# PlantandFoodResearch/MCHap

Measured on AMD Instinct MI355X. Metric: loci/sec (whole node) for 1000-step MCMC, tetraploid 8-SNV loci, 1/2/4/8 GPUs, higher is better.
Workload: dtype f64; 1 GPU; 10000 synthetic tetraploid loci per GPU, 8 SNVs, 200 reads, 1000 MCMC steps x 2 chains, burn 500, posterior summary (BASELINE.json configs[1]); 4 passes in flight on separate HIP streams, each with its own device buffers; loci_per_gpu=10000, ploidy=4, snvs=8, reads=200, mcmc_steps=1000, chains=2, burn=500, llk_cache=True, passes_in_flight=4, hw_queues=4, world_size=1, devices=1

## Files before the change

include/mchap_hip.h:

```cpp
#ifndef MCHAP_HIP_H
#define MCHAP_HIP_H

#include <stdint.h>
#include <stddef.h>

#ifdef __cplusplus
extern "C" {
#endif

#define MCHAP_MAX_TEMPS 16
#define MCHAP_MAX_PLOIDY 8
#define MCHAP_MAX_PLOIDY_DENOVO 15
#define MCHAP_MAX_POS 126
#define MCHAP_MAX_ALLELE 8
#define MCHAP_MAX_READS 4096

enum {
  MCHAP_OK = 0,
  MCHAP_ERR_NAN_LLK = -1,
  MCHAP_ERR_BAD_ARG = -2,
  MCHAP_ERR_BREAKS = -3,
  MCHAP_ERR_LIMIT = -4,
  MCHAP_ERR_HIP = -5,
  MCHAP_ERR_NO_DEVICE = -6
// ... 57 lines not shown
  uint64_t stream_id;
  int32_t initial_n_het;
  int32_t reserved;
} mchap_unit;

int mchap_denovo_fit_batch_device(const mchap_denovo_cfg *cfg, int n_units, const mchap_unit *units_dev,
                                  const mchap_unit *units_host, const double *reads, const int64_t *read_counts,
                                  const int8_t *n_alleles, const int8_t *initial, uint64_t *trace_words,
                                  double *llks, int8_t *fixed_alleles, int32_t *status, void *workspace,
                                  int64_t workspace_bytes, void *stream);

int mchap_denovo_fit_batch_calls_device(const mchap_denovo_cfg *cfg, int n_units, const mchap_unit *units_dev,
                                        const mchap_unit *units_host, const int8_t *calls, const int16_t *quals,
                                        const double *qual_prob, int qual_prob_len, const int64_t *read_counts,
                                        const int8_t *n_alleles, const int8_t *initial, uint64_t *trace_words,
                                        double *llks, int8_t *fixed_alleles, int32_t *status, void *workspace,
                                        int64_t workspace_bytes, void *stream);

int64_t mchap_denovo_workspace_bytes(const mchap_denovo_cfg *cfg, int n_units, const mchap_unit *units_host);

int mchap_denovo_fit_batch(const mchap_denovo_cfg *cfg, int n_units, const mchap_unit *units,
                           const double *reads, int64_t reads_len, const int64_t *read_counts, int64_t counts_len,
                           const int8_t *n_alleles, int64_t nalleles_len, const int8_t *initial, int64_t initial_len,
                           uint64_t *trace_words, int64_t trace_len, double *llks, int64_t llks_len,
                           int8_t *fixed_alleles, int64_t fixed_len, int32_t *status);

int mchap_log_likelihood_batch(const double *reads, int n_reads, int n_pos, int max_allele,
                               const int64_t *read_counts, const int8_t *genotypes, int n_genotypes, int ploidy,
                               double *llks_out);

int mchap_read_log_batch(const double *x, int64_t n, double *out);
int mchap_read_log_product_batch(const double *x, int64_t n, int group, double *out);
int mchap_wave_sum_batch(const double *x, int64_t n_waves, double *out);

int mchap_trace_posterior_batch_device(int n_units, const mchap_unit *units_dev, int steps, int chains, int burn,
                                       const uint64_t *trace_words, int max_states, int ploidy_max,
                                       uint64_t *post_words, int32_t *post_counts, int32_t *post_n,
                                       double *mode_stats, int32_t *mode_index, uint64_t *mode_words,
                                       int32_t *mode_count, void *stream);

int mchap_trace_posterior_max_states(int ploidy_max);
int mchap_trace_posterior_listed_device(int n_list, const int32_t *unit_list_dev, const mchap_unit *units_dev, int steps, int chains,
                                        int burn, const uint64_t *trace_words, int cap, int ploidy_max, uint64_t *post_words,
                                        int32_t *post_counts, int32_t *post_n, double *mode_stats, int32_t *mode_index,
                                        uint64_t *mode_words, int32_t *mode_count, void *stream);

int mchap_call_incongruence_batch_device(int n_units, const mchap_unit *units_dev, int steps, int chains, int burn,
                                         const int64_t *genotypes, int ploidy_max, double threshold, int32_t *mci, void *stream);
int mchap_call_incongruence_listed_device(int n_list, const int32_t *unit_list_dev, const mchap_unit *units_dev, int steps, int chains,
                                          int burn, const int64_t *genotypes, int cap, int ploidy_max, double threshold, int32_t *mci,
                                          void *stream);

int mchap_exact_genotype_likelihoods(const double *reads, int n_reads, int n_pos, int max_allele,
                                     const int64_t *read_counts, const int8_t *haplotypes, int n_haps, int ploidy,
                                     float *llks_out, double *llks64_out);

int mchap_exact_genotype_posteriors(const void *llks, int is_f32, int64_t n_genotypes, int ploidy, int n_alleles,
                                    int has_prior, double inbreeding, const double *frequencies, double *post_out);

int mchap_trace_incongruence_batch_device(int n_units, const mchap_unit *units_dev, int steps, int chains, int burn,
                                          const uint64_t *trace_words, int ploidy_max, double threshold, int32_t *mci,
                                          void *stream);

int mchap_trace_incongruence_listed_device(int n_list, const int32_t *unit_list_dev, const mchap_unit *units_dev, int steps, int chains,
                                           int burn, const uint64_t *trace_words, int cap, int ploidy_max, double threshold, int32_t *mci,
                                           void *stream);
// ... 97 lines not shown
```

mchap_amd/_lib.py:

```python
import ctypes as C
import os
import threading
import subprocess

import numpy as np

HERE = os.path.dirname(os.path.abspath(__file__))
CSRC = os.path.join(HERE, "csrc")
SO = os.environ.get("MCHAP_HIP_LIB") or os.path.join(CSRC, "libmchap_hip.so")
TEST_SO = os.path.join(CSRC, "libmchap_hip_test.so")

MAX_TEMPS = 16
MAX_PLOIDY = 8
MAX_PLOIDY_GENERAL = 15
MAX_ALLELE = 8
MAX_READS = 4096

OK = 0
ERR_NAN_LLK = -1
ERR_BAD_ARG = -2
ERR_BREAKS = -3
ERR_LIMIT = -4
ERR_HIP = -5
ERR_NO_DEVICE = -6
# ... 213 lines not shown
    "mchap_trace_posterior_batch_wph_device",
    "mchap_trace_posterior_max_states_wph",
    "mchap_trace_posterior_listed_wph_device",
    "mchap_trace_incongruence_batch_wph_device",
    "mchap_trace_incongruence_listed_wph_device",
    "mchap_call_incongruence_batch_device",
    "mchap_call_incongruence_listed_device",
    "mchap_exact_genotype_likelihoods",
    "mchap_exact_genotype_posteriors",
    "mchap_exact_posterior_mode_batch",
    "mchap_exact_workspace_bytes",
    "mchap_exact_workspace_bytes_cached",
    "mchap_exact_call_batch_device",
    "mchap_exact_posterior_summaries_batch_device",
    "mchap_exact_posterior_summaries",
    "mchap_call_mcmc_workspace_bytes",
    "mchap_call_mcmc_workspace_bytes_for",
    "mchap_call_mcmc_max_haps",
    "mchap_call_mcmc_batch_device",
    "mchap_call_mcmc_batch",
    "mchap_call_reads_from_calls_device",
    "mchap_version",
    "mchap_last_error",
    "mchap_device_count",
    "mchap_denovo_lds_bytes",
    "mchap_denovo_workspace_bytes",
    "mchap_timer_create",
    "mchap_timer_ms",
    "mchap_timer_destroy",
    "mchap_denovo_sampler_name",
    "mchap_read_log_batch",
    "mchap_read_log_product_batch",
    "mchap_wave_sum_batch",
    "mchap_denovo_trace_words_per_haplotype",
]


def last_error():
    return lib().mchap_last_error().decode()


def check(rc):
    if rc == OK:
        return
    msg = last_error()
    if rc == ERR_NAN_LLK:
        raise ValueError("Encountered log likelihood of nan")
    if rc == ERR_BREAKS:
        raise ValueError("breaks must be smaller then n")
    if rc == ERR_BAD_ARG:
        raise AssertionError(msg)
    if rc == ERR_LIMIT:
        raise NotImplementedError("mchap_hip: " + msg)
    raise MchapLibraryError("mchap_hip error %d: %s" % (rc, msg))


def ptr(a):
    return None if a is None else C.c_void_p(a.ctypes.data)
```

mchap_amd/csrc/denovo_coast_kernel.hpp:

```cpp
#pragma once
#include "denovo_spec_kernel.hpp"

namespace mchap {

template <int NW>
__device__ __forceinline__ void coast_chain(const SimtParams &P, unsigned char *smem, int slot) {
  const DenovoParams &D = P.d;
  const int tid = threadIdx.x;
  const int lane = tid & (WAVE - 1), wv = tid / WAVE;
  constexpr int NT = NW * WAVE;
  auto block_sync = [] {
    if constexpr (NW == 1) lds_sync();
    else __syncthreads();
  };
  const int Cn = D.chains, Sn = D.steps, mmax = P.max_pos;
  const int E = spec_memo_entries(mmax);
  const long long q = P.pipe_list ? (long long)P.pipe_list[slot] : (long long)slot;
  PipeState *st = reinterpret_cast<PipeState *>(P.pipe_state) + q;
  const int base = st->step;
  if (base >= Sn) return;
  const int u = (int)(q / Cn), chain = (int)(q % Cn);
  const mchap_unit U = D.units[u];
  const int32_t *mi = P.meta_i + (size_t)u * meta_i_stride(P.max_pos);
  const int K = U.ploidy;
  const int Mh = mi[META_I_MH];
  const int n = K * Mh;
  if (st->mvalid == 0 || n > spec_draws(K, mmax)) {
    if (tid == 0) P.pipe_out[atomicAdd(P.pipe_out_count, 1)] = (int32_t)q;
    return;
  }
  LDSP(double) mt = lds_cast<double>(smem);
  LDSP(double) bc = mt + 2 * E;
  LDSP(uint64_t) tw = lds_cast<uint64_t>(smem + (size_t)8 * (2 * E + mmax));
  LDSP(int) wfail = lds_cast<int>(smem + (size_t)8 * (2 * E + mmax + 8));
  const double mlo = st->mlo, mhi = st->mhi;
  {
    const double *pm = P.pipe_memo + (size_t)q * 2 * E;
    for (int i = tid; i < 2 * E; i += NT) mt[i] = pm[i];
  }
  if (tid == 0) {
    if (D.n_intervals == 0) {
      double cacc = 0.0;
      for (int j = 0; j < Mh; j++) {
        cacc += D.break_table[(size_t)Mh * D.max_pos + j];
        bc[j] = cacc;
      }
    }
    uint64_t w[8];
#pragma unroll
    for (int h = 0; h < 8; h++) w[h] = h < K ? st->g[h] : ~0ull;
#pragma unroll
    for (int pass = 0; pass < 8; pass++) {
#pragma unroll
      for (int i = pass & 1; i + 1 < 8; i += 2) {
        const uint64_t a = w[i], b = w[i + 1];
        w[i] = a < b ? a : b;
        w[i + 1] = a < b ? b : a;
      }
    }
#pragma unroll
    for (int h = 0; h < 8; h++) tw[h] = w[h];
  }
  block_sync();
  Stream s;
  s.k0 = (uint32_t)D.seed;
  s.k1 = (uint32_t)(D.seed >> 32) ^ (uint32_t)(U.stream_id >> 32);
  s.c2 = ((uint32_t)chain << 16) | 0u;
  s.c3 = (uint32_t)U.stream_id;
  int stop = Sn;
  int sweep = 0;
  for (int s0 = base; s0 < Sn; s0 += NT, sweep++) {
    const int step = s0 + tid;
    bool fail = false;
    if (step < Sn) {
      const uint64_t ctr0 = (uint64_t)step * STEP_DRAWS;
      const uint64_t ub = ctr0 + (uint64_t)(n - 1), ue = ub + (uint64_t)n;
      uint64_t dblk = ~0ull, dw0 = 0, dw1 = 0;
      auto words_at = [&](uint64_t d) -> uint64_t {
        const uint64_t b = d >> 1;
        if (b != dblk) {
          uint32_t o[4];
          philox4x32_10((uint32_t)b, (uint32_t)(b >> 32), s.c2, s.c3, s.k0, s.k1, o);
          dw0 = (uint64_t)o[0] | ((uint64_t)o[1] << 32);
          dw1 = (uint64_t)o[2] | ((uint64_t)o[3] << 32);
          dblk = b;
        }
        return (d & 1) ? dw1 : dw0;
      };
      bool ok = true;
      for (uint64_t b = ub >> 1; 2 * b < ue; b++) {
        uint32_t o[4];
        philox4x32_10((uint32_t)b, (uint32_t)(b >> 32), s.c2, s.c3, s.k0, s.k1, o);
        const uint64_t d0 = 2 * b;
        const uint64_t w0 = (uint64_t)o[0] | ((uint64_t)o[1] << 32), w1 = (uint64_t)o[2] | ((uint64_t)o[3] << 32);
        if (d0 >= ub && d0 < ue) {
          const double x = draw_double(w0);
          ok = ok && (mlo <= x) && (x < mhi);
        }
        if (d0 + 1 >= ub && d0 + 1 < ue) {
          const double x = draw_double(w1);
          ok = ok && (mlo <= x) && (x < mhi);
        }
        dblk = b;
        dw0 = w0;
        dw1 = w1;
      }
      fail = !ok;
      uint64_t ctr = ue;
      for (int kind = 0; kind < 3 && !fail; kind++) {
        const double pstep = kind == 0 ? D.p_recomb : (kind == 1 ? D.p_partial : D.p_dosage);
        const bool doit = draw_double(words_at(ctr)) <= pstep;
        ctr++;
        if (!doit) continue;
        uint64_t zeros;
        int n_int;
        if (kind < 2) {
          int nb;
          if (D.n_intervals > 0) {
            ctr++;
            nb = D.n_intervals - 1;
          } else {
            const double x = draw_double(words_at(ctr));
            ctr++;
            nb = Mh;
            for (int j = Mh - 1; j >= 0; j--)
              if (bc[j] > x) nb = j;
          }
          if (nb >= Mh) {
            fail = true;
            break;
          }
          uint64_t ind = ((1ull << Mh) - 1ull) & ~1ull;
          for (int b = 0; b < nb; b++) {
            const int no = __popcll(ind);
            if (no == 0) break;
            int k = 0;
            if (no > 1) {
              k = (int)draw_interval(words_at(ctr), (uint32_t)(no - 1));
              ctr++;
            }
            uint64_t t = ind;
            while (k-- > 0) t &= t - 1;
            ind &= ~(t & (~t + 1));
          }
          zeros = ~ind & ((1ull << (Mh + 1)) - 1ull);
          n_int = nb + 1;
        } else {
          zeros = 1ull | (1ull << Mh);
          n_int = 1;
        }
        LDSP(double) mtot = mt + (kind == 0 ? 0 : E);
        if (n_int == 1) {
          const double tot = mtot[spec_memo_index(0, Mh)];
          if (tot < 0.0) continue;
          if (!(draw_double(words_at(ctr)) >= tot)) {
            fail = true;
            break;
          }
          ctr++;
        } else {
          double mx = -1.0;
          int n_cons = 0;
          bool unknown = false;
          uint64_t z = zeros;
          int start = __ffsll((long long)z) - 1;
          z &= z - 1;
          for (int i = 0; i < n_int; i++) {
            const int stop_ = __ffsll((long long)z) - 1;
            z &= z - 1;
            const double tot = mtot[spec_memo_index(start, stop_)];
            if (isnan(tot)) unknown = true;
            else if (tot >= 0.0) {
              n_cons++;
              mx = fmax(mx, tot);
            }
            start = stop_;
          }
          bool low = unknown;
          for (int k = 0; k < n_cons && !low; k++)
            low = !(draw_double(words_at(ctr + (uint64_t)(n_int - 1 + k))) >= mx);
          if (low) {
            fail = true;
            break;
          }
          ctr += (uint64_t)(n_int - 1 + n_cons);
        }
      }
    }
    const unsigned long long fb = __ballot(fail);
    if constexpr (NW == 1) {
      if (fb) {
        stop = s0 + __ffsll((long long)fb) - 1;
        break;
      }
    } else {
      LDSP(int) wf = wfail + (sweep & 1) * NW;
      if (lane == 0) wf[wv] = fb ? s0 + wv * WAVE + __ffsll((long long)fb) - 1 : Sn;
      __syncthreads();
      int first = Sn;
#pragma unroll
      for (int w = 0; w < NW; w++) first = min(first, wf[w]);
      if (first < Sn) {
        stop = first;
        break;
      }
    }
  }
  if (tid == 0) {
    st->step = stop;
    if (stop < Sn) P.pipe_out[atomicAdd(P.pipe_out_count, 1)] = (int32_t)q;
  }
  const int rows = stop - base;
  uint64_t *tp = D.trace + U.trace_off + (size_t)chain * D.steps * K + (size_t)base * K;
  uint64_t *lp = reinterpret_cast<uint64_t *>(D.llks + U.llk_off + (size_t)chain * D.steps) + base;
  const int nw = rows * K;
  int h = tid % K;
  const int hs = NT % K;
  for (int i = tid; i < nw; i += NT) {
    tp[i] = tw[h];
// ... 23 lines not shown
```

mchap_amd/csrc/denovo_spec_kernel.hpp:

```cpp
#pragma once
#include <type_traits>

#include "denovo_simt_kernel.hpp"

#ifdef MCHAP_MASK_PADDING
#define MCHAP_PAD_LANE(x) (x)
#else
#define MCHAP_PAD_LANE(x) true
#endif
#ifndef MCHAP_COOP_UNR
#define MCHAP_COOP_UNR 2
#endif
#ifndef MCHAP_SPEC_TB
#define MCHAP_SPEC_TB 4
#endif
#ifndef MCHAP_SPEC_LOW
#define MCHAP_SPEC_LOW 8
#endif
#ifndef MCHAP_SPEC_CG
#define MCHAP_SPEC_CG 4
#endif
#ifndef MCHAP_SPEC_VAR
#define MCHAP_SPEC_VAR 0
#endif
#define MCHAP_SPEC_SBS (MCHAP_SPEC_VAR == 1)
#define MCHAP_SPEC_DEEP (MCHAP_SPEC_VAR == 2)
#ifndef MCHAP_SPEC_WIN0
#define MCHAP_SPEC_WIN0 4
#endif
#ifndef MCHAP_SPEC_WIN_MIN
#define MCHAP_SPEC_WIN_MIN 2
#endif
#ifndef MCHAP_REUSE_MAXK
#define MCHAP_REUSE_MAXK 8
#endif
#ifndef MCHAP_CODED_UNR
#define MCHAP_CODED_UNR 16
#endif

namespace mchap {

constexpr int SPEC_MAX_IV = 64;
constexpr int SPEC_TB = MCHAP_SPEC_TB;
constexpr int SPEC_LN = 72;
constexpr int SPEC_DRAWS_MAX = 384;
__host__ __device__ inline int spec_draws(int K, int Mmax) {
  int d = 2 * K * Mmax - 1;
  if (d < 3 * Mmax + 2) d = 3 * Mmax + 2;
  d = (d + 1) & ~1;
  return d < SPEC_DRAWS_MAX ? d : SPEC_DRAWS_MAX;
}

#define LDSP(T) __attribute__((address_space(3))) T *
#define GLBP(T) __attribute__((address_space(1))) T *
template <class T>
__device__ __forceinline__ LDSP(T) lds_cast(void *p) {
  return (LDSP(T))p;
}

template <bool LT>
struct TabPtr;
template <>
struct TabPtr<false> {
  typedef GLBP(const uint8_t) u8;
  typedef GLBP(const double) f64;
  template <class CT>
  static __device__ __forceinline__ CT ld(u8 p) { return *reinterpret_cast<GLBP(const CT)>(p); }
};
template <>
struct TabPtr<true> {
  typedef LDSP(const uint8_t) u8;
  typedef LDSP(const double) f64;
  template <class CT>
  static __device__ __forceinline__ CT ld(u8 p) { return *reinterpret_cast<LDSP(const CT)>(p); }
};

enum { GP_RT = 0, GP_CW, GP_CT, GP_CACHE, GP_CKEYS, GP_TRACE, GP_LLK, GP_GBP, GP_N };
// ... 59 lines not shown
  const size_t per_group = (size_t)2 * spec_memo_entries(Mmax) * 8;
  if (T != 1 || per_group > 16 * 1024) return 0;
  return per_group * (64 / G);
}

constexpr int SPEC_LC_ENTRIES = 256;
#ifndef MCHAP_LC_GEN
#define MCHAP_LC_GEN 48
#endif
constexpr uint32_t SPEC_LC_SECOND_LEVEL_GEN = MCHAP_LC_GEN;
__host__ __device__ inline size_t spec_lc_bytes(int entries = SPEC_LC_ENTRIES) { return (size_t)16 * entries + 16; }
__host__ __device__ inline bool spec_ctx_in_bpc(int K, int Mmax, int Amax, int max_reads) {
  return K >= 3 && max_reads <= 64 && Mmax * Amax <= 24 * (K - 2) && 16 * K * Mmax <= 3 * 64 * 8 && 12 * 64 + 4 * 8 <= 3 * 64 * 8;
}
__host__ __device__ inline int spec_lc_entries(int bp_cache) { return (bp_cache & 2) ? ((bp_cache & 4) ? SPEC_LC_ENTRIES / 2 : SPEC_LC_ENTRIES) : 0; }
__device__ __forceinline__ uint32_t sct_off(uint32_t row) { return (row / 24u) * (uint32_t)(4 * WAVE * 8) + (row % 24u) * (uint32_t)WAVE; }
__host__ __device__ inline size_t spec_bp_cache_bytes(int K) { return (size_t)8 * K * 4 * 64 + (size_t)8 * (K + 1); }

constexpr int COAST_NW_LIST = 4;
__host__ __device__ inline size_t coast_lds_bytes(int Mmax) {
  return (size_t)8 * (2 * spec_memo_entries(Mmax) + Mmax) + (size_t)8 * 12;
}

__host__ __device__ inline size_t spec_lds_bytes(int K, int Mmax, int Amax, int T, int G) {
  const int NG = 64 / G;
  const int nmax = K * Mmax;
  const int nopt = Amax > 1 ? Amax - 1 : 1;
  const int niv = Mmax + 1;
  size_t b = 0;
  b += (size_t)8 * K * 64;
  b += (size_t)8 * NG * T * K;
  b += (size_t)8 * NG * T * 2;
  b += (size_t)8 * NG * (2 * K + 5);
  b += (size_t)8 * 64;
  b += (size_t)8 * nopt * 64 * 2;
  b += (size_t)8 * SPEC_LN * 2;
  b += (size_t)8 * NG * Mmax;
  b += (size_t)4 * NG * niv * 4;
  b += (size_t)2 * NG * Mmax;
  b += (size_t)2 * NG * nmax;
  b += (size_t)NG * Mmax * 2;
  b += (size_t)NG * nmax;
  b += (size_t)NG * niv;
  b = (b + 1) & ~(size_t)1;
  b += (size_t)2 * NG * 2;
  b = (b + 15) & ~(size_t)15;
  b += (size_t)8 * NG * DICT_MAX;
  b += (size_t)8 * NG * GP_N;
  b += (size_t)8 * NG * GV_N;
  b = (b + 15) & ~(size_t)15;
  b += (size_t)16 * NG;
  b += (size_t)8 * NG * K;
  b += (size_t)8 * NG * (K + 1);
  b += (size_t)8 * NG * SPEC_TB * (K + 1);
  b = (b + 15) & ~(size_t)15;
  b += (size_t)8 * NG * spec_draws(K, Mmax);
  b += spec_memo_bytes(Mmax, T, G);
  return (b + 63) & ~(size_t)63;
}

struct Stream {
  uint32_t k0, k1, c2, c3;
};
__device__ __forceinline__ void stream_words(const Stream &s, uint64_t n, uint32_t &a, uint32_t &b) {
  uint32_t o[4];
  const uint64_t blk = n >> 1;
  philox4x32_10((uint32_t)blk, (uint32_t)(blk >> 32), s.c2, s.c3, s.k0, s.k1, o);
  a = (n & 1) ? o[2] : o[0];
  b = (n & 1) ? o[3] : o[1];
}
__device__ __forceinline__ double stream_double(const Stream &s, uint64_t n) {
  uint32_t a, b;
  stream_words(s, n, a, b);
  return ((double)(a >> 5) * 67108864.0 + (double)(b >> 6)) * (1.0 / 9007199254740992.0);
}
__device__ __forceinline__ uint32_t stream_interval(const Stream &s, uint64_t n, uint32_t max) {
  uint32_t a, b;
  stream_words(s, n, a, b);
  return __umulhi(a, max + 1u);
}

template <int G>
__device__ __forceinline__ void stage_draws(const Stream &s, uint64_t base, int count, LDSP(uint64_t) tab, int gl, bool active) {
  if (active) {
    const uint64_t b0 = base >> 1;
    const int nblk = (int)(((base + (uint64_t)count + 1) >> 1) - b0);
    for (int b = gl; b < nblk; b += G) {
      uint32_t o[4];
      const uint64_t blk = b0 + (uint64_t)b;
      philox4x32_10((uint32_t)blk, (uint32_t)(blk >> 32), s.c2, s.c3, s.k0, s.k1, o);
      const long long i0 = (long long)(blk << 1) - (long long)base;
      if (i0 >= 0 && i0 < count) tab[i0] = (uint64_t)o[0] | ((uint64_t)o[1] << 32);
      if (i0 + 1 >= 0 && i0 + 1 < count) tab[i0 + 1] = (uint64_t)o[2] | ((uint64_t)o[3] << 32);
    }
  }
}
__device__ __forceinline__ double draw_double(uint64_t w) {
  return ((double)((uint32_t)w >> 5) * 67108864.0 + (double)((uint32_t)(w >> 32) >> 6)) * (1.0 / 9007199254740992.0);
}
__device__ __forceinline__ uint32_t draw_interval(uint64_t w, uint32_t max) { return __umulhi((uint32_t)w, max + 1u); }

template <int G>
__device__ __forceinline__ uint64_t grp_ballot(bool p, int gi) {
  const unsigned long long m = __ballot(p);
  if (G == 64) return m;
  return (m >> (gi * G)) & ((1ull << G) - 1ull);
}
__device__ __forceinline__ bool wave_any(bool p) { return __ballot(p) != 0ull; }

template <int CTRL>
__device__ __forceinline__ double dpp_f64(double v) {
  const long long b = __double_as_longlong(v);
  const int lo = __builtin_amdgcn_update_dpp(0, (int)(unsigned)b, CTRL, 0xf, 0xf, false);
  const int hi = __builtin_amdgcn_update_dpp(0, (int)(unsigned)((unsigned long long)b >> 32), CTRL, 0xf, 0xf, false);
  return __longlong_as_double((long long)(((unsigned long long)(unsigned)hi << 32) | (unsigned)lo));
}
template <int G>
__device__ __forceinline__ double grp_max_f64(double v) {
#pragma unroll
  for (int o = G / 2; o >= 16; o >>= 1) v = fmax(v, __shfl_xor(v, o, G));
  v = fmax(v, dpp_f64<0x128>(v));
  v = fmax(v, dpp_f64<0x124>(v));
  v = fmax(v, dpp_f64<0x122>(v));
  v = fmax(v, dpp_f64<0x121>(v));
  return v;
}
__device__ __forceinline__ void lds_sync() {
#ifdef MCHAP_SYNC_BARRIER
  __syncthreads();
#else
  __builtin_amdgcn_fence(__ATOMIC_ACQ_REL, "workgroup");
  __builtin_amdgcn_wave_barrier();
#endif
// ... 1889 lines not shown
          const int idx = spec_memo_index((int)(se & 255u), (int)(se >> 8));
          mtot[idx] = no > 0 ? cacc : -1.0;
          ctx_tot(idx, no > 0 ? cacc : -1.0);
        }
        off += no;
      }
      ii0 = ii;
    }
    {
      const int src = acc_gl >= 0 ? acc_gl : 0;
      GWords<KT> nw;
#pragma unroll
      for (int h = 0; h < KT; h++) nw.w[h] = __shfl(pw.w[h], src, G);
      const double nl = __shfl(llk_i, src, G);
      if (acc_gl >= 0) {
        c.g = nw;
        c.llk = nl;
        genotype_changed<KT>(c);
      }
    }
    if (!done && ii0 >= n_int) done = true;
    lds_sync();
  }
  } while (fill && wave_any(filling && n_int > 0));
  GPHASE(c, 7);
  return ok;
}



constexpr int SPEC_TW_MAX = 8;
__host__ __device__ inline size_t spec_tw_exchange_bytes(int K, int T) { return (((size_t)8 * T * (K + 1) + 16) + 63) & ~(size_t)63; }

template <int KT, int G, bool PIPE = false, int VAR = MCHAP_SPEC_VAR, bool TW = false, bool CTX = false>
__global__ __launch_bounds__(TW ? 64 * SPEC_TW_MAX : 64, TW ? 2 : MCHAP_SPEC_WPE) void denovo_spec_kernel(const SimtParams P) {
  extern __shared__ __align__(16) unsigned char smem_all[];
  constexpr int NG = 64 / G;
  const DenovoParams &D = P.d;
  const int lane = threadIdx.x & (WAVE - 1);
  const int tw = TW ? (int)(threadIdx.x / WAVE) : 0;
  unsigned char *smem = smem_all + (TW ? spec_tw_exchange_bytes(KT, D.n_temps) + (size_t)tw * (size_t)P.tw_lds : 0);
  LDSP(uint64_t) xw = lds_cast<uint64_t>(smem_all);
  LDSP(double) xllk = lds_cast<double>(smem_all + (size_t)8 * D.n_temps * KT);
  LDSP(int) xdead = lds_cast<int>(smem_all + (size_t)8 * D.n_temps * (KT + 1));
  if (TW && threadIdx.x == 0) *xdead = 0;
  const int gi = lane / G, gl = lane % G;
  int n_list = 0;
  long long my_slot = (long long)blockIdx.x * NG + gi;
  int parts_eff = 1, my_part = 0;
  const bool fillonly = PIPE && (P.pipe_mode & PIPE_FILLONLY);
  if constexpr (PIPE) {
    n_list = P.pipe_count ? *P.pipe_count : (int)((long long)P.n_units * D.chains);
    parts_eff = pipe_parts_eff(n_list, P.pipe_parts);
    if (fillonly) {
      if (parts_eff <= 1) return;
      const int n_slots = n_list * parts_eff;
      const int n_waves = min(n_slots, (int)gridDim.x);
      if ((int)blockIdx.x >= n_waves) return;
      const long long v = (long long)gi * n_waves + blockIdx.x;
      my_slot = v < n_slots ? v / parts_eff : (long long)n_list;
      my_part = (int)(v % parts_eff);
    } else if (P.pipe_list) {
      const int n_waves = min(n_list, (int)gridDim.x);
      if ((int)blockIdx.x >= n_waves) return;
      my_slot = (long long)gi * n_waves + blockIdx.x;
    } else if ((long long)blockIdx.x * NG >= n_list) {
      return;
    }
  }
  const int T = PIPE ? 1 : D.n_temps;
  const int Cn = D.chains, Sn = D.steps;
  const int mmax = P.max_pos, nmax = KT * P.max_pos;
  const int rpad = D.rpad;
  SpecLds S;
  {
    const int nopt = P.max_allele > 1 ? P.max_allele - 1 : 1;
    const int niv = mmax + 1;
    unsigned char *p = smem;
    S.pw = lds_cast<uint64_t>(p); p += (size_t)8 * KT * 64;
    S.wst = lds_cast<uint64_t>(p); p += (size_t)8 * NG * T * KT;
    S.llk_t = lds_cast<double>(p); p += (size_t)8 * NG * T;
    S.rngn = lds_cast<uint64_t>(p); p += (size_t)8 * NG * T;
    S.prior = lds_cast<double>(p); p += (size_t)8 * NG * (2 * KT + 5);
    S.ptab = lds_cast<double>(p); p += (size_t)8 * 64;
    S.optp = lds_cast<double>(p); p += (size_t)8 * nopt * 64;
    S.optl = lds_cast<double>(p); p += (size_t)8 * nopt * 64;
    S.ln = lds_cast<double>(p); p += (size_t)8 * SPEC_LN;
    S.lninv = lds_cast<double>(p); p += (size_t)8 * SPEC_LN;
    S.bdist = lds_cast<double>(p); p += (size_t)8 * NG * mmax;
    S.ivse = lds_cast<uint32_t>(p); p += (size_t)4 * NG * niv;
    S.ivlin = lds_cast<uint32_t>(p); p += (size_t)4 * NG * niv;
    S.ivlout = lds_cast<uint32_t>(p); p += (size_t)4 * NG * niv;
    S.ivno = lds_cast<uint32_t>(p); p += (size_t)4 * NG * niv;
    S.cols = lds_cast<uint16_t>(p); p += (size_t)2 * NG * mmax;
    S.permtab = lds_cast<uint16_t>(p); p += (size_t)2 * NG * nmax;
    S.shift = lds_cast<uint8_t>(p); p += (size_t)NG * mmax;
    S.nal = lds_cast<uint8_t>(p); p += (size_t)NG * mmax;
    S.ktab = lds_cast<uint8_t>(p); p += (size_t)NG * nmax;
    S.ordtab = lds_cast<uint8_t>(p); p += (size_t)NG * niv;
    p = smem + (((size_t)(p - smem) + 1) & ~(size_t)1);
    S.nreads = lds_cast<uint16_t>(p); p += (size_t)2 * NG;
    S.ndict = lds_cast<uint16_t>(p); p += (size_t)2 * NG;
    p = smem + (((size_t)(p - smem) + 15) & ~(size_t)15);
    S.dict = lds_cast<double>(p); p += (size_t)8 * NG * DICT_MAX;
    S.gptr = lds_cast<uint64_t>(p); p += (size_t)8 * NG * GP_N;
    S.gval = lds_cast<double>(p); p += (size_t)8 * NG * GV_N;
    p = smem + (((size_t)(p - smem) + 15) & ~(size_t)15);
    S.gstream = lds_cast<uint32_t>(p); p += (size_t)16 * NG;
    S.bw = lds_cast<uint64_t>(p); p += (size_t)8 * NG * KT;
    S.gbt = lds_cast<uint64_t>(p); p += (size_t)8 * NG * (KT + 1);
    for (int i = lane; i < NG * (KT + 1); i += WAVE) S.gbt[i] = 0ull;
    S.tbuf = lds_cast<uint64_t>(p); p += (size_t)8 * NG * SPEC_TB * (KT + 1);
    p = smem + (((size_t)(p - smem) + 15) & ~(size_t)15);
    S.ndraws = spec_draws(KT, mmax);
    S.draws = lds_cast<uint64_t>(p); p += (size_t)8 * NG * S.ndraws;
    S.memo_stride = (spec_memo_bytes(mmax, T, G) && !(P.flags & 2)) ? 2 * spec_memo_entries(mmax) : 0;
    S.memo_tot = lds_cast<double>(p);
    for (int i = lane; i < NG * S.memo_stride; i += WAVE) S.memo_tot[i] = NAN;
    S.bpc = nullptr;
    S.bpt = nullptr;
    S.lc = lds_cast<uint64_t>(p);
// ... 4 lines not shown
      S.bpc = lds_cast<double>(p); p += (size_t)8 * KT * 4 * 64;
      S.bpt = lds_cast<uint64_t>(p); p += (size_t)8 * (KT + 1);
      if (lane == 0) S.bpt[KT] = 0ull;
      if (P.bp_cache & 2) {
        p = smem + (((size_t)(p - smem) + 15) & ~(size_t)15);
        S.lc = lds_cast<uint64_t>(p);
        const int lce = spec_lc_entries(P.bp_cache);
        S.lc_mask = (uint32_t)lce - 1u;
        for (int i = lane; i < 2 * lce; i += WAVE) S.lc[i] = 0ull;
        p += spec_lc_bytes(lce);
      }
    } else {
      p += spec_memo_bytes(mmax, T, G);
    }
    if constexpr (CTX && G == 64 && PIPE) {
      if (P.ctx != nullptr && P.ctx_n > 0) {
        if (P.bp_cache & 8) {
          S.cx_lds = (LDSP(unsigned char))(S.bpc + (size_t)((KT - 1) * 4 + 1) * WAVE);
          S.cx_val = S.bpc + (size_t)((KT - 2) * 4 + 1) * WAVE;
        } else {
          p = smem + (((size_t)(p - smem) + 15) & ~(size_t)15);
          S.cx_lds = lds_cast<unsigned char>(p); p += (size_t)12 * SPEC_CTX_MAX + 4 * CX_N;
          S.cx_val = lds_cast<double>(p); p += (size_t)16 * nmax;
        }
        S.cx_n = P.ctx_n < SPEC_CTX_MAX ? P.ctx_n : SPEC_CTX_MAX;
        if (lane < CX_N) CXP_ST(S)[lane] = 0u;
        if (lane < SPEC_CTX_MAX) {
          CXP_TAG(S)[lane] = 0ull;
          CXP_STAMP(S)[lane] = 0u;
        }
      }
    }
  }
  for (int i = lane; i < SPEC_LN; i += WAVE) {
    S.ln[i] = c_ln[i];
    S.lninv[i] = c_ln_inv[i];
  }
  long long q = my_slot;
  const long long n_chains = (long long)P.n_units * Cn;
  Grp<KT> c;
  c.alive = q < n_chains;
  bool listed = false;
  if constexpr (PIPE) {
    listed = q < n_list;
    c.alive = listed;
    if (listed && P.pipe_list) q = P.pipe_list[q];
    if (!listed) q = 0;
  }
  const bool resume = PIPE && (P.pipe_mode & PIPE_RESUME);
  int base = 0;
  const int u = c.alive ? (int)(q / Cn) : 0;
  const int chain = c.alive ? (int)(q % Cn) : 0;
  const mchap_unit U = D.units[u];
  const int32_t *mi = P.meta_i + (size_t)u * meta_i_stride(P.max_pos);
  const double *mf = P.meta_f + (size_t)u * meta_f_stride(P.max_ploidy, P.max_pos, P.max_allele);
  if (c.alive && mi[META_I_STATUS] != MCHAP_UNIT_OK) c.alive = false;
  const int A = U.max_allele;
  c.Mh = c.alive ? mi[META_I_MH] : 1;
  c.bits = allele_bits(A);
  c.flat = c.alive && mi[META_I_FLAT] != 0 && !(P.flags & 128);
  if (gl == 0) {
    S.gval[gi * GV_N + GV_INB] = U.inbreeding;
    S.gval[gi * GV_N + GV_MLO] = 0.0;
    S.gval[gi * GV_N + GV_MHI] = 0.0;
    S.gstream[gi * 4 + 0] = (uint32_t)D.seed;
    S.gstream[gi * 4 + 1] = (uint32_t)(D.seed >> 32) ^ (uint32_t)(U.stream_id >> 32);
    S.gstream[gi * 4 + 2] = ((uint32_t)chain << 16) | 0u;
// ... 387 lines not shown
#if defined(MCHAP_STATS) || defined(MCHAP_PHASES)
      if (threadIdx.x == 0)
        for (int i_ = 0; i_ < 12; i_++) atomicAdd(&g_stats[36 + i_], c.ph[i_]);
#endif
      if (fillonly) {
        if (listed && c.alive) {
          double *pm = P.pipe_memo + (size_t)q * S.memo_stride;
          for (int i = gl; i < S.memo_stride; i += G)
            if (i % parts_eff == my_part) pm[i] = S.memo_tot[gi * S.memo_stride + i];
        }
      } else if (listed) {
        PipeState *st = reinterpret_cast<PipeState *>(P.pipe_state) + q;
        const GWords<KT> ge = c.g;
        if (gl == 0) {
#pragma unroll
          for (int h = 0; h < KT; h++) st->g[h] = ge.w[h];
          st->llk = c.llk;
          st->ctr = c.ctr;
          st->mlo = S.gval[gi * GV_N + GV_MLO];
          st->mhi = S.gval[gi * GV_N + GV_MHI];
          st->mvalid = (c.alive && c.mvalid && c.memo_on) ? 1 : 0;
          st->step = c.alive ? base + n_done : Sn;
        }
        if (c.alive) {
          double *pm = P.pipe_memo + (size_t)q * S.memo_stride;
          for (int i = gl; i < S.memo_stride; i += G) pm[i] = S.memo_tot[gi * S.memo_stride + i];
        }
      }
    }
  }
  if (status != MCHAP_UNIT_OK && gl == 0) atomicMax(&D.status[u], status);
}

}
```

mchap_amd/csrc/mchap_hip.hip:

```cpp
#include <hip/hip_runtime.h>

#include <cmath>
#include <cstdarg>
#include <cstdio>
#include <cstdlib>
#include <cstring>
#include <algorithm>
#include <atomic>
#include <mutex>
#include <vector>

#include "../../include/mchap_hip.h"
#include "denovo_kernel.hpp"
#include "denovo_simt_kernel.hpp"
#include "denovo_spec_kernel.hpp"
#include "denovo_fillw_kernel.hpp"
#ifdef MCHAP_TEST_KERNELS
#include "denovo_fill_kernel.hpp"
#include "denovo_lane_kernel.hpp"
#endif
#include "exact_kernel.hpp"
#include "call_mcmc_kernel.hpp"
#include "posterior_kernel.hpp"

// ... 1275 lines not shown
  if (rc) return rc;
  if (n <= 0) return MCHAP_OK;
  if (!x || !out || group < 1 || group > 4) return fail(MCHAP_ERR_BAD_ARG, "NULL buffer or group not in 1..4");
  DevBuf d_x, d_o;
  HostCall hc;
  MCHAP_TRY(hc.open());
  HIP_TRY(hipMalloc(&d_x.p, (size_t)n * group * 8));
  HIP_TRY(hipMalloc(&d_o.p, (size_t)n * 8));
  MCHAP_TRY(hc.up(d_x.p, x, (size_t)n * group * 8));
  hipLaunchKernelGGL(mchap::read_log_product_kernel, dim3((unsigned)std::min<int64_t>((n + 255) / 256, 4096)), dim3(256), 0, hc.stream,
                     d_x.as<double>(), (long long)n, group, d_o.as<double>());
  HIP_TRY(hipGetLastError());
  MCHAP_TRY(hc.down(out, d_o.p, (size_t)n * 8));
  return hc.sync();
}

int mchap_wave_sum_batch(const double *x, int64_t n_waves, double *out) {
  int rc = ensure_init();
  if (rc) return rc;
  if (n_waves <= 0) return MCHAP_OK;
  if (!x || !out) return fail(MCHAP_ERR_BAD_ARG, "NULL buffer");
  DevBuf d_x, d_o;
  HostCall hc;
  MCHAP_TRY(hc.open());
  HIP_TRY(hipMalloc(&d_x.p, (size_t)n_waves * 64 * 8));
  HIP_TRY(hipMalloc(&d_o.p, (size_t)n_waves * 8));
  MCHAP_TRY(hc.up(d_x.p, x, (size_t)n_waves * 64 * 8));
  hipLaunchKernelGGL(mchap::wave_sum_kernel, dim3((unsigned)n_waves), dim3(64), 0, hc.stream, d_x.as<double>(), d_o.as<double>());
  HIP_TRY(hipGetLastError());
  MCHAP_TRY(hc.down(out, d_o.p, (size_t)n_waves * 8));
  return hc.sync();
}

#include "api_posterior_exact.inc"

}
```

mchap_amd/csrc/spec_inst.hip:

```cpp
#include <hip/hip_runtime.h>

#include "../../include/mchap_hip.h"
#include "denovo_spec_kernel.hpp"

#define SPEC_CAT_(a, k, g) a##k##_##g
#define SPEC_CAT(a, k, g) SPEC_CAT_(a, k, g)

#ifdef SPEC_PIPE
#if MCHAP_SPEC_VAR == 1
#define mchap_specp_init_ mchap_specs_init_
#define mchap_specp_launch_ mchap_specs_launch_
#define mchap_specp_launchc_ mchap_specs_launchc_
#define mchap_specp_stats_ mchap_specs_stats_
#elif MCHAP_SPEC_VAR == 2
#define mchap_specp_init_ mchap_specd_init_
#define mchap_specp_launch_ mchap_specd_launch_
#define mchap_specp_launchc_ mchap_specd_launchc_
#define mchap_specp_stats_ mchap_specd_stats_
#endif
extern "C" __attribute__((visibility("hidden"))) int SPEC_CAT(mchap_specp_init_, SPEC_K, SPEC_G)(const double *ln,
                                                                                                 const double *ln_inv) {
  if (hipMemcpyToSymbol(HIP_SYMBOL(mchap::c_ln), ln, sizeof(double) * 260) != hipSuccess) return 1;
  if (hipMemcpyToSymbol(HIP_SYMBOL(mchap::c_ln_inv), ln_inv, sizeof(double) * 260) != hipSuccess) return 1;
  return 0;
}

extern "C" __attribute__((visibility("hidden"))) int SPEC_CAT(mchap_specp_launch_, SPEC_K, SPEC_G)(
    const mchap::SimtParams *P, unsigned grid, size_t lds, hipStream_t stream) {
  auto ks = mchap::denovo_spec_kernel<SPEC_K, SPEC_G, true>;
  if (lds > 64 * 1024) {
    const hipError_t e = hipFuncSetAttribute(reinterpret_cast<const void *>(ks), hipFuncAttributeMaxDynamicSharedMemorySize, (int)lds);
    if (e != hipSuccess) return (int)e;
  }
  hipLaunchKernelGGL(ks, dim3(grid), dim3(64), lds, stream, *P);
  return (int)hipGetLastError();
}

#if SPEC_G == 64
extern "C" __attribute__((visibility("hidden"))) int SPEC_CAT(mchap_specp_launchc_, SPEC_K, SPEC_G)(
    const mchap::SimtParams *P, unsigned grid, size_t lds, hipStream_t stream) {
  auto ks = mchap::denovo_spec_kernel<SPEC_K, SPEC_G, true, MCHAP_SPEC_VAR, false, true>;
  if (lds > 64 * 1024) {
    const hipError_t e = hipFuncSetAttribute(reinterpret_cast<const void *>(ks), hipFuncAttributeMaxDynamicSharedMemorySize, (int)lds);
    if (e != hipSuccess) return (int)e;
  }
  hipLaunchKernelGGL(ks, dim3(grid), dim3(64), lds, stream, *P);
  return (int)hipGetLastError();
}
#endif
#else
extern "C" __attribute__((visibility("hidden"))) int SPEC_CAT(mchap_spec_init_, SPEC_K, SPEC_G)(const double *ln,
                                                                                                const double *ln_inv) {
  if (hipMemcpyToSymbol(HIP_SYMBOL(mchap::c_ln), ln, sizeof(double) * 260) != hipSuccess) return 1;
  if (hipMemcpyToSymbol(HIP_SYMBOL(mchap::c_ln_inv), ln_inv, sizeof(double) * 260) != hipSuccess) return 1;
  return 0;
}

extern "C" __attribute__((visibility("hidden"))) int SPEC_CAT(mchap_spec_launch_, SPEC_K, SPEC_G)(
    const mchap::SimtParams *P, unsigned grid, size_t lds, hipStream_t stream) {
  auto ks = mchap::denovo_spec_kernel<SPEC_K, SPEC_G>;
  if (lds > 64 * 1024) {
    const hipError_t e = hipFuncSetAttribute(reinterpret_cast<const void *>(ks), hipFuncAttributeMaxDynamicSharedMemorySize, (int)lds);
// ... 36 lines not shown
```

Before: 1.113 million loci/s.

## Rewrite coast chain checks with integer u53 thresholds and a flat state machine

The coast kernel now turns the memo totals, break cumulatives, move probabilities and acceptance bounds into 53-bit integer thresholds once, then compares raw integer draws against them instead of converting each draw to double. The per-step decision logic becomes a non-unrolled state machine that walks the Philox blocks one at a time with 32-bit counters, replacing nested loops and a lambda cache. The aim is to cut f64 conversion work, 64-bit counter math and divergence in the per-thread speculative check. A host test entry point is added to compare float and integer decisions, since the threshold rounding must match the old semantics exactly, including NaN and boundary cases.

```diff
diff --git a/include/mchap_hip.h b/include/mchap_hip.h
--- a/include/mchap_hip.h
+++ b/include/mchap_hip.h
@@ -113,6 +113,8 @@
 int mchap_read_log_batch(const double *x, int64_t n, double *out);
 int mchap_read_log_product_batch(const double *x, int64_t n, int group, double *out);
 int mchap_wave_sum_batch(const double *x, int64_t n_waves, double *out);
+int mchap_draw_decisions_batch(const double *lo, const double *hi, const uint32_t *w0, const uint32_t *w1, int64_t n,
+                               uint8_t *f64_out, uint8_t *u53_out);
 
 int mchap_trace_posterior_batch_device(int n_units, const mchap_unit *units_dev, int steps, int chains, int burn,
                                        const uint64_t *trace_words, int max_states, int ploidy_max,
diff --git a/mchap_amd/_lib.py b/mchap_amd/_lib.py
--- a/mchap_amd/_lib.py
+++ b/mchap_amd/_lib.py
@@ -269,6 +269,7 @@
     "mchap_read_log_batch",
     "mchap_read_log_product_batch",
     "mchap_wave_sum_batch",
+    "mchap_draw_decisions_batch",
     "mchap_denovo_trace_words_per_haplotype",
 ]
 
diff --git a/mchap_amd/csrc/denovo_coast_kernel.hpp b/mchap_amd/csrc/denovo_coast_kernel.hpp
--- a/mchap_amd/csrc/denovo_coast_kernel.hpp
+++ b/mchap_amd/csrc/denovo_coast_kernel.hpp
@@ -2,6 +2,14 @@
 #include "denovo_spec_kernel.hpp"
 
 namespace mchap {
+
+constexpr uint64_t COAST_NONE = ~0ull;
+enum { COAST_LAST, COAST_DOIT, COAST_BREAKS, COAST_PICK, COAST_STAY, COAST_DONE };
+
+__device__ __forceinline__ uint64_t coast_uniform(uint64_t v) {
+  return (uint64_t)(uint32_t)__builtin_amdgcn_readfirstlane((int)(uint32_t)v) |
+         ((uint64_t)(uint32_t)__builtin_amdgcn_readfirstlane((int)(uint32_t)(v >> 32)) << 32);
+}
 
 template <int NW>
 __device__ __forceinline__ void coast_chain(const SimtParams &P, unsigned char *smem, int slot) {
@@ -29,21 +37,26 @@
     if (tid == 0) P.pipe_out[atomicAdd(P.pipe_out_count, 1)] = (int32_t)q;
     return;
   }
-  LDSP(double) mt = lds_cast<double>(smem);
-  LDSP(double) bc = mt + 2 * E;
+  LDSP(uint64_t) mt = lds_cast<uint64_t>(smem);
+  LDSP(uint64_t) bc = mt + 2 * E;
   LDSP(uint64_t) tw = lds_cast<uint64_t>(smem + (size_t)8 * (2 * E + mmax));
   LDSP(int) wfail = lds_cast<int>(smem + (size_t)8 * (2 * E + mmax + 8));
-  const double mlo = st->mlo, mhi = st->mhi;
+  const uint64_t tlo = coast_uniform(u53_threshold(st->mlo)), thi = coast_uniform(u53_threshold(st->mhi, 0));
+  const uint64_t tp0 = coast_uniform(u53_threshold_above(D.p_recomb, 0)), tp1 = coast_uniform(u53_threshold_above(D.p_partial, 0)),
+                 tp2 = coast_uniform(u53_threshold_above(D.p_dosage, 0));
   {
     const double *pm = P.pipe_memo + (size_t)q * 2 * E;
-    for (int i = tid; i < 2 * E; i += NT) mt[i] = pm[i];
+    for (int i = tid; i < 2 * E; i += NT) {
+      const double tot = pm[i];
+      mt[i] = tot < 0.0 ? COAST_NONE : u53_threshold(tot);
+    }
   }
   if (tid == 0) {
     if (D.n_intervals == 0) {
       double cacc = 0.0;
       for (int j = 0; j < Mh; j++) {
         cacc += D.break_table[(size_t)Mh * D.max_pos + j];
-        bc[j] = cacc;
+        bc[j] = u53_threshold(cacc, 0);
       }
     }
     uint64_t w[8];
@@ -67,124 +80,106 @@
   s.k1 = (uint32_t)(D.seed >> 32) ^ (uint32_t)(U.stream_id >> 32);
   s.c2 = ((uint32_t)chain << 16) | 0u;
   s.c3 = (uint32_t)U.stream_id;
+  static_assert(STEP_DRAWS == 65536, "block counter of a step: (step >> 17, step << 15 | offset)");
+  const uint32_t blast = (uint32_t)(n - 1);
   int stop = Sn;
   int sweep = 0;
   for (int s0 = base; s0 < Sn; s0 += NT, sweep++) {
     const int step = s0 + tid;
     bool fail = false;
     if (step < Sn) {
-      const uint64_t ctr0 = (uint64_t)step * STEP_DRAWS;
-      const uint64_t ub = ctr0 + (uint64_t)(n - 1), ue = ub + (uint64_t)n;
-      uint64_t dblk = ~0ull, dw0 = 0, dw1 = 0;
-      auto words_at = [&](uint64_t d) -> uint64_t {
-        const uint64_t b = d >> 1;
-        if (b != dblk) {
-          uint32_t o[4];
-          philox4x32_10((uint32_t)b, (uint32_t)(b >> 32), s.c2, s.c3, s.k0, s.k1, o);
-          dw0 = (uint64_t)o[0] | ((uint64_t)o[1] << 32);
-          dw1 = (uint64_t)o[2] | ((uint64_t)o[3] << 32);
-          dblk = b;
-        }
-        return (d & 1) ? dw1 : dw0;
-      };
+      const uint32_t c0 = (uint32_t)step << 15, c1 = (uint32_t)step >> 17;
+      uint64_t w0 = 0, w1 = 0;
       bool ok = true;
-      for (uint64_t b = ub >> 1; 2 * b < ue; b++) {
+      for (uint32_t b = (uint32_t)(n - 1) >> 1; b < blast; b++) {
         uint32_t o[4];
-        philox4x32_10((uint32_t)b, (uint32_t)(b >> 32), s.c2, s.c3, s.k0, s.k1, o);
-        const uint64_t d0 = 2 * b;
-        const uint64_t w0 = (uint64_t)o[0] | ((uint64_t)o[1] << 32), w1 = (uint64_t)o[2] | ((uint64_t)o[3] << 32);
-        if (d0 >= ub && d0 < ue) {
-          const double x = draw_double(w0);
-          ok = ok && (mlo <= x) && (x < mhi);
-        }
-        if (d0 + 1 >= ub && d0 + 1 < ue) {
-          const double x = draw_double(w1);
-          ok = ok && (mlo <= x) && (x < mhi);
-        }
-        dblk = b;
-        dw0 = w0;
-        dw1 = w1;
-      }
+        philox4x32_10(c0 + b, c1, s.c2, s.c3, s.k0, s.k1, o);
+        const uint64_t x0 = draw_u53((uint64_t)o[0] | ((uint64_t)o[1] << 32)), x1 = draw_u53((uint64_t)o[2] | ((uint64_t)o[3] << 32));
+        const bool whole = 2 * b >= (uint32_t)(n - 1);
+        ok = ok && x0 >= (whole ? tlo : 0ull) && x0 < (whole ? thi : U53_ONE) && x1 >= tlo && x1 < thi;
+      }
+      int state = ok ? COAST_LAST : COAST_DONE;
       fail = !ok;
-      uint64_t ctr = ue;
-      for (int kind = 0; kind < 3 && !fail; kind++) {
-        const double pstep = kind == 0 ? D.p_recomb : (kind == 1 ? D.p_partial : D.p_dosage);
-        const bool doit = draw_double(words_at(ctr)) <= pstep;
-        ctr++;
-        if (!doit) continue;
-        uint64_t zeros;
-        int n_int;
-        if (kind < 2) {
-          int nb;
-          if (D.n_intervals > 0) {
-            ctr++;
-            nb = D.n_intervals - 1;
-          } else {
-            const double x = draw_double(words_at(ctr));
-            ctr++;
+      uint32_t d = 2 * blast, blk = ~0u;
+      int kind = 0, nb = 0, left = 0, rem = 0;
+      uint64_t ind = 0, mx = 0;
+#pragma nounroll
+      for (;;) {
+#pragma nounroll
+        while (state != COAST_DONE && (d >> 1) == blk) {
+          const uint64_t w = (d & 1) ? w1 : w0;
+          const uint64_t x = draw_u53(w);
+          d++;
+          bool pick = false, next = false;
+          if (state == COAST_LAST) {
+            if (x >= tlo && x < thi) state = COAST_DOIT;
+            else fail = true;
+          } else if (state == COAST_DOIT) {
+            if (!(x < (kind == 0 ? tp0 : (kind == 1 ? tp1 : tp2)))) next = true;
+            else if (kind == 2) {
+              nb = 0;
+              pick = true;
+            } else if (D.n_intervals > 0) {
+              d++;
+              nb = D.n_intervals - 1;
+              pick = true;
+            } else state = COAST_BREAKS;
+          } else if (state == COAST_BREAKS) {
             nb = Mh;
             for (int j = Mh - 1; j >= 0; j--)
-              if (bc[j] > x) nb = j;
-          }
-          if (nb >= Mh) {
-            fail = true;
-            break;
-          }
-          uint64_t ind = ((1ull << Mh) - 1ull) & ~1ull;
-          for (int b = 0; b < nb; b++) {
-            const int no = __popcll(ind);
-            if (no == 0) break;
-            int k = 0;
-            if (no > 1) {
-              k = (int)draw_interval(words_at(ctr), (uint32_t)(no - 1));
-              ctr++;
-            }
+              if (x < bc[j]) nb = j;
+            pick = true;
+          } else if (state == COAST_PICK) {
+            int k = (int)draw_interval(w, (uint32_t)(__popcll(ind) - 1));
             uint64_t t = ind;
             while (k-- > 0) t &= t - 1;
             ind &= ~(t & (~t + 1));
-          }
-          zeros = ~ind & ((1ull << (Mh + 1)) - 1ull);
-          n_int = nb + 1;
-        } else {
-          zeros = 1ull | (1ull << Mh);
-          n_int = 1;
+            left--;
+          } else {
+            if (x < mx) fail = true;
+            else if (--rem == 0) next = true;
+          }
+          if (pick) {
+            if (kind < 2 && nb >= Mh) fail = true;
+            ind = ((1ull << Mh) - 1ull) & ~1ull;
+            left = nb;
+            state = COAST_PICK;
+          }
+          if (state == COAST_PICK && !(left > 0 && __popcll(ind) > 1) && !fail) {
+            if (left > 0) ind = 0;
+            const int n_int = nb + 1;
+            LDSP(uint64_t) mtot = mt + (kind == 0 ? 0 : E);
+            uint64_t z = ~ind & ((1ull << (Mh + 1)) - 1ull);
+            int start = __ffsll((long long)z) - 1;
+            z &= z - 1;
+            rem = 0;
+            mx = 0;
+            for (int i = 0; i < n_int; i++) {
+              const int stop_ = __ffsll((long long)z) - 1;
+              z &= z - 1;
+              const uint64_t t = mtot[spec_memo_index(start, stop_)];
+              if (t != COAST_NONE) {
+                rem++;
+                mx = t > mx ? t : mx;
+              }
+              start = stop_;
+            }
+            d += (uint32_t)(n_int - 1);
+            if (rem == 0) next = true;
+            else state = COAST_STAY;
+          }
+          if (next) {
+            kind++;
+            state = kind == 3 ? COAST_DONE : COAST_DOIT;
+          }
+          if (fail) state = COAST_DONE;
         }
-        LDSP(double) mtot = mt + (kind == 0 ? 0 : E);
-        if (n_int == 1) {
-          const double tot = mtot[spec_memo_index(0, Mh)];
-          if (tot < 0.0) continue;
-          if (!(draw_double(words_at(ctr)) >= tot)) {
-            fail = true;
-            break;
-          }
-          ctr++;
-        } else {
-          double mx = -1.0;
-          int n_cons = 0;
-          bool unknown = false;
-          uint64_t z = zeros;
-          int start = __ffsll((long long)z) - 1;
-          z &= z - 1;
-          for (int i = 0; i < n_int; i++) {
-            const int stop_ = __ffsll((long long)z) - 1;
-            z &= z - 1;
-            const double tot = mtot[spec_memo_index(start, stop_)];
-            if (isnan(tot)) unknown = true;
-            else if (tot >= 0.0) {
-              n_cons++;
-              mx = fmax(mx, tot);
-            }
-            start = stop_;
-          }
-          bool low = unknown;
-          for (int k = 0; k < n_cons && !low; k++)
-            low = !(draw_double(words_at(ctr + (uint64_t)(n_int - 1 + k))) >= mx);
-          if (low) {
-            fail = true;
-            break;
-          }
-          ctr += (uint64_t)(n_int - 1 + n_cons);
-        }
+        if (state == COAST_DONE) break;
+        blk = d >> 1;
+        uint32_t o[4];
+        philox4x32_10(c0 + blk, c1, s.c2, s.c3, s.k0, s.k1, o);
+        w0 = (uint64_t)o[0] | ((uint64_t)o[1] << 32);
+        w1 = (uint64_t)o[2] | ((uint64_t)o[3] << 32);
       }
     }
     const unsigned long long fb = __ballot(fail);
diff --git a/mchap_amd/csrc/denovo_spec_kernel.hpp b/mchap_amd/csrc/denovo_spec_kernel.hpp
--- a/mchap_amd/csrc/denovo_spec_kernel.hpp
+++ b/mchap_amd/csrc/denovo_spec_kernel.hpp
@@ -235,6 +235,22 @@
   return ((double)((uint32_t)w >> 5) * 67108864.0 + (double)((uint32_t)(w >> 32) >> 6)) * (1.0 / 9007199254740992.0);
 }
 __device__ __forceinline__ uint32_t draw_interval(uint64_t w, uint32_t max) { return __umulhi((uint32_t)w, max + 1u); }
+constexpr uint64_t U53_ONE = 1ull << 53;
+__device__ __forceinline__ uint64_t draw_u53(uint64_t w) {
+  return ((uint64_t)((uint32_t)w >> 5) << 26) | (uint64_t)((uint32_t)(w >> 32) >> 6);
+}
+__device__ __forceinline__ uint64_t u53_threshold(double t, uint64_t nan = U53_ONE) {
+  if (t != t) return nan;
+  if (!(t > 0.0)) return 0ull;
+  if (t >= 1.0) return U53_ONE;
+  return (uint64_t)ceil(t * 9007199254740992.0);
+}
+__device__ __forceinline__ uint64_t u53_threshold_above(double t, uint64_t nan = U53_ONE) {
+  if (t != t) return nan;
+  if (t < 0.0) return 0ull;
+  if (t >= 1.0) return U53_ONE;
+  return (uint64_t)floor(t * 9007199254740992.0) + 1ull;
+}
 
 template <int G>
 __device__ __forceinline__ uint64_t grp_ballot(bool p, int gi) {
diff --git a/mchap_amd/csrc/mchap_hip.hip b/mchap_amd/csrc/mchap_hip.hip
--- a/mchap_amd/csrc/mchap_hip.hip
+++ b/mchap_amd/csrc/mchap_hip.hip
@@ -1331,6 +1331,48 @@
   return hc.sync();
 }
 
+namespace mchap {
+static __global__ void draw_decisions_kernel(const double *lo, const double *hi, const uint32_t *w0, const uint32_t *w1, long long n,
+                                             uint8_t *f64_out, uint8_t *u53_out) {
+  for (long long i = (long long)blockIdx.x * blockDim.x + threadIdx.x; i < n; i += (long long)gridDim.x * blockDim.x) {
+    const uint64_t w = (uint64_t)w0[i] | ((uint64_t)w1[i] << 32);
+    const double x = draw_double(w);
+    const uint64_t u = draw_u53(w);
+    f64_out[i] = (uint8_t)((lo[i] <= x ? 1 : 0) | (x < hi[i] ? 2 : 0) | (x <= hi[i] ? 4 : 0));
+    u53_out[i] = (uint8_t)((u >= u53_threshold(lo[i]) ? 1 : 0) | (u < u53_threshold(hi[i], 0) ? 2 : 0) |
+                           (u < u53_threshold_above(hi[i], 0) ? 4 : 0));
+  }
+}
+}
+
+int mchap_draw_decisions_batch(const double *lo, const double *hi, const uint32_t *w0, const uint32_t *w1, int64_t n,
+                               uint8_t *f64_out, uint8_t *u53_out) {
+  int rc = ensure_init();
+  if (rc) return rc;
+  if (n <= 0) return MCHAP_OK;
+  if (!lo || !hi || !w0 || !w1 || !f64_out || !u53_out) return fail(MCHAP_ERR_BAD_ARG, "NULL buffer");
+  DevBuf d_lo, d_hi, d_w0, d_w1, d_f, d_u;
+  HostCall hc;
+  MCHAP_TRY(hc.open());
+  HIP_TRY(hipMalloc(&d_lo.p, (size_t)n * 8));
+  HIP_TRY(hipMalloc(&d_hi.p, (size_t)n * 8));
+  HIP_TRY(hipMalloc(&d_w0.p, (size_t)n * 4));
+  HIP_TRY(hipMalloc(&d_w1.p, (size_t)n * 4));
+  HIP_TRY(hipMalloc(&d_f.p, (size_t)n));
+  HIP_TRY(hipMalloc(&d_u.p, (size_t)n));
+  MCHAP_TRY(hc.up(d_lo.p, lo, (size_t)n * 8));
+  MCHAP_TRY(hc.up(d_hi.p, hi, (size_t)n * 8));
+  MCHAP_TRY(hc.up(d_w0.p, w0, (size_t)n * 4));
+  MCHAP_TRY(hc.up(d_w1.p, w1, (size_t)n * 4));
+  hipLaunchKernelGGL(mchap::draw_decisions_kernel, dim3((unsigned)std::min<int64_t>((n + 255) / 256, 4096)), dim3(256), 0, hc.stream,
+                     d_lo.as<double>(), d_hi.as<double>(), d_w0.as<uint32_t>(), d_w1.as<uint32_t>(), (long long)n, d_f.as<uint8_t>(),
+                     d_u.as<uint8_t>());
+  HIP_TRY(hipGetLastError());
+  MCHAP_TRY(hc.down(f64_out, d_f.p, (size_t)n));
+  MCHAP_TRY(hc.down(u53_out, d_u.p, (size_t)n));
+  return hc.sync();
+}
+
 #include "api_posterior_exact.inc"
 
 }
```

Result: slower. 1.015 million loci/s (-8.8%).

## Add register-capped pipelined spec kernel and shrink LDS tables to needed size

Applied to the files above, without the earlier changes.

Splits the spec kernel into a shared body and adds a separate pipelined entry point for G=64 that caps VGPRs through amdgpu_num_vgpr, so more waves can be resident per SIMD. It also sizes the ln/ln_inv LDS tables by K instead of a fixed 72 entries, aliases ptab onto optp, and drops the optl table when there is only one option. The goal is lower LDS and register footprint and higher occupancy, at the risk of register spills in the capped kernel and subtle aliasing bugs if ptab and optp are live at the same time.

```diff
diff --git a/mchap_amd/csrc/denovo_spec_kernel.hpp b/mchap_amd/csrc/denovo_spec_kernel.hpp
--- a/mchap_amd/csrc/denovo_spec_kernel.hpp
+++ b/mchap_amd/csrc/denovo_spec_kernel.hpp
@@ -43,6 +43,10 @@
 constexpr int SPEC_MAX_IV = 64;
 constexpr int SPEC_TB = MCHAP_SPEC_TB;
 constexpr int SPEC_LN = 72;
+__host__ __device__ inline int spec_ln_entries(int K) {
+  const int n = K * (K - 1) > 8 ? K * (K - 1) : 8;
+  return (n + 2) & ~1;
+}
 constexpr int SPEC_DRAWS_MAX = 384;
 __host__ __device__ inline int spec_draws(int K, int Mmax) {
   int d = 2 * K * Mmax - 1;
@@ -168,9 +172,9 @@
   b += (size_t)8 * NG * T * K;
   b += (size_t)8 * NG * T * 2;
   b += (size_t)8 * NG * (2 * K + 5);
-  b += (size_t)8 * 64;
-  b += (size_t)8 * nopt * 64 * 2;
-  b += (size_t)8 * SPEC_LN * 2;
+  b += (size_t)8 * nopt * 64;
+  if (nopt > 1) b += (size_t)8 * nopt * 64;
+  b += (size_t)8 * spec_ln_entries(K) * 2;
   b += (size_t)8 * NG * Mmax;
   b += (size_t)4 * NG * niv * 4;
   b += (size_t)2 * NG * Mmax;
@@ -2190,8 +2194,8 @@
 constexpr int SPEC_TW_MAX = 8;
 __host__ __device__ inline size_t spec_tw_exchange_bytes(int K, int T) { return (((size_t)8 * T * (K + 1) + 16) + 63) & ~(size_t)63; }
 
-template <int KT, int G, bool PIPE = false, int VAR = MCHAP_SPEC_VAR, bool TW = false, bool CTX = false>
-__global__ __launch_bounds__(TW ? 64 * SPEC_TW_MAX : 64, TW ? 2 : MCHAP_SPEC_WPE) void denovo_spec_kernel(const SimtParams P) {
+template <int KT, int G, bool PIPE, bool TW, bool CTX>
+__device__ __forceinline__ void denovo_spec_body(const SimtParams &P) {
   extern __shared__ __align__(16) unsigned char smem_all[];
   constexpr int NG = 64 / G;
   const DenovoParams &D = P.d;
@@ -2240,11 +2244,15 @@
     S.llk_t = lds_cast<double>(p); p += (size_t)8 * NG * T;
     S.rngn = lds_cast<uint64_t>(p); p += (size_t)8 * NG * T;
     S.prior = lds_cast<double>(p); p += (size_t)8 * NG * (2 * KT + 5);
-    S.ptab = lds_cast<double>(p); p += (size_t)8 * 64;
+    S.ptab = lds_cast<double>(p);
     S.optp = lds_cast<double>(p); p += (size_t)8 * nopt * 64;
-    S.optl = lds_cast<double>(p); p += (size_t)8 * nopt * 64;
-    S.ln = lds_cast<double>(p); p += (size_t)8 * SPEC_LN;
-    S.lninv = lds_cast<double>(p); p += (size_t)8 * SPEC_LN;
+    if (nopt > 1) {
+      S.optl = lds_cast<double>(p); p += (size_t)8 * nopt * 64;
+    } else {
+      S.optl = lds_cast<double>(smem);
+    }
+    S.ln = lds_cast<double>(p); p += (size_t)8 * spec_ln_entries(KT);
+    S.lninv = lds_cast<double>(p); p += (size_t)8 * spec_ln_entries(KT);
     S.bdist = lds_cast<double>(p); p += (size_t)8 * NG * mmax;
     S.ivse = lds_cast<uint32_t>(p); p += (size_t)4 * NG * niv;
     S.ivlin = lds_cast<uint32_t>(p); p += (size_t)4 * NG * niv;
@@ -2315,7 +2323,7 @@
       }
     }
   }
-  for (int i = lane; i < SPEC_LN; i += WAVE) {
+  for (int i = lane; i < spec_ln_entries(KT); i += WAVE) {
     S.ln[i] = c_ln[i];
     S.lninv[i] = c_ln_inv[i];
   }
@@ -2769,4 +2777,18 @@
   if (status != MCHAP_UNIT_OK && gl == 0) atomicMax(&D.status[u], status);
 }
 
-}
+template <int KT, int G, bool PIPE = false, int VAR = MCHAP_SPEC_VAR, bool TW = false, bool CTX = false>
+__global__ __launch_bounds__(TW ? 64 * SPEC_TW_MAX : 64, TW ? 2 : MCHAP_SPEC_WPE) void denovo_spec_kernel(const SimtParams P) {
+  denovo_spec_body<KT, G, PIPE, TW, CTX>(P);
+}
+
+#ifndef MCHAP_SPEC_FIRST_VGPRS
+#define MCHAP_SPEC_FIRST_VGPRS 232
+#endif
+constexpr int SPEC_FIRST_VGPRS = MCHAP_SPEC_FIRST_VGPRS;
+template <int KT, int VAR = MCHAP_SPEC_VAR>
+__global__ __launch_bounds__(64, MCHAP_SPEC_WPE) __attribute__((amdgpu_num_vgpr(MCHAP_SPEC_FIRST_VGPRS / 2))) void denovo_spec_first_kernel(const SimtParams P) {
+  denovo_spec_body<KT, 64, true, false, false>(P);
+}
+
+}
diff --git a/mchap_amd/csrc/spec_inst.hip b/mchap_amd/csrc/spec_inst.hip
--- a/mchap_amd/csrc/spec_inst.hip
+++ b/mchap_amd/csrc/spec_inst.hip
@@ -27,7 +27,11 @@
 
 extern "C" __attribute__((visibility("hidden"))) int SPEC_CAT(mchap_specp_launch_, SPEC_K, SPEC_G)(
     const mchap::SimtParams *P, unsigned grid, size_t lds, hipStream_t stream) {
+#if SPEC_G == 64 && MCHAP_SPEC_VAR == 0
+  auto ks = mchap::denovo_spec_first_kernel<SPEC_K>;
+#else
   auto ks = mchap::denovo_spec_kernel<SPEC_K, SPEC_G, true>;
+#endif
   if (lds > 64 * 1024) {
     const hipError_t e = hipFuncSetAttribute(reinterpret_cast<const void *>(ks), hipFuncAttributeMaxDynamicSharedMemorySize, (int)lds);
     if (e != hipSuccess) return (int)e;
```

Result: no change. 1.113 million loci/s before, 1.116 million loci/s after (median of 6 runs) (+0.3%).
